# zengyan-97/X2-VLM

Measured on AMD Instinct MI355X. Metric: image-text pairs/sec (fwd+bwd) X2VLM-base 224px bs=64/GPU, higher is better.
Workload: dtype bf16

## Files before the change

### x2-vlm_amd/csrc/gemm.hip

```cpp
#include "x2_common.h"
#include <type_traits>

#define BM 128
#define BN 128
#define BK 64
#define TILE_BYTES (128 * 128)
#define STAGE_BYTES (2 * TILE_BYTES)
#define GEMM_LDS_BYTES (2 * STAGE_BYTES)

struct GemmNT {
  const bf16_t* A; const bf16_t* B; void* C;
  const float* bias; const float* gamma; const float* resid; bf16_t* aux;
  int M, N, K;
  int lda, ldb, ldc, ldr, ldaux;
  int act;
  int out_f32;
  int group_m;
  DropSpec drop;
  const uint32_t* drop_epoch;
  const float* rowscale;
  float* colsum;
  int dbg;
  int ksplit;
  const long* ce_labels;
// ... 1054 lines not shown
    const bool use64 = g_tune[3] == 3 || (g_tune[3] == 0 && (t128 <= slots || (t128 <= slots + slots / 6 && K <= 1024)));
    const bool use192 = !use64 && (g_tune[3] == 2 || (g_tune[3] == 0 && t128 > slots && t192 <= slots));
    const int t160 = ((M + 159) / 160) * ((N + BN - 1) / BN);
    const bool use160 = g_tune[3] == 4 || (use192 && g_tune[3] == 0 && t160 <= slots);
#define X2_NT_LAUNCH(V, SW)                                                                          \
    do {                                                                                              \
      if (use64) launch_nt<2, V, SW>(p, t64, (hipStream_t)stream);                                    \
      else if (use160) launch_nt<5, V, SW>(p, t160, (hipStream_t)stream);                             \
      else if (use192) launch_nt<6, V, SW>(p, t192, (hipStream_t)stream);                             \
      else launch_nt<4, V, SW>(p, t128, (hipStream_t)stream);                                         \
    } while (0)
    switch (var) {
      case 0: X2_NT_LAUNCH(0, false); break;
      case 2: X2_NT_LAUNCH(2, false); break;
      case 3: X2_NT_LAUNCH(3, false); break;
      case 1: X2_NT_LAUNCH(1, true); break;
      case 5: X2_NT_LAUNCH(5, true); break;
      case 6: X2_NT_LAUNCH(6, true); break;
      default: X2_NT_LAUNCH(4, false); break;
    }
#undef X2_NT_LAUNCH
  }
  return x2_check_launch("x2_gemm_nt");
}

extern "C" int x2_gemm_nt_dgelu_colparts(const void* A, const void* B, void* C, int M, int N, int K, int lda, int ldb, int ldc,
                                         const void* aux, int ldaux, float* colparts, int* nrows_out, void* stream) {
  X2_REQUIRE(A && B && C && aux && colparts && nrows_out, "x2_gemm_nt_dgelu_colparts: null argument");
  X2_REQUIRE(M > 0 && N > 0 && K > 0 && K % BK == 0 && N % 8 == 0, "x2_gemm_nt_dgelu_colparts: M=%d N=%d K=%d", M, N, K);
  X2_REQUIRE(lda % 8 == 0 && ldb % 8 == 0 && ldc % 8 == 0 && ldaux % 8 == 0, "x2_gemm_nt_dgelu_colparts: leading dims must keep 16-byte rows");
  GemmNT p{(const bf16_t*)A, (const bf16_t*)B, C, nullptr, nullptr, nullptr, (bf16_t*)aux, M, N, K, lda, ldb, ldc, 0, ldaux, 2, 0,
           g_tune[0] > 0 ? g_tune[0] : 8, DropSpec{0u, 0u, 1.f}, nullptr, nullptr, colparts, 0, 0};
  const int tiles_n = (N + BN - 1) / BN, t128 = ((M + 127) / 128) * tiles_n, t192 = ((M + 191) / 192) * tiles_n, t64 = ((M + 63) / 64) * tiles_n;
  const int slots = 2 * x2_cus();
  const bool use64 = g_tune[3] == 3 || (g_tune[3] == 0 && (t128 <= slots || (t128 <= slots + slots / 6 && K <= 1024)));
  const bool use192 = !use64 && (g_tune[3] == 2 || (g_tune[3] == 0 && t128 > slots && t192 <= slots));
  if (use64) { launch_nt<2, 10, false>(p, t64, (hipStream_t)stream); *nrows_out = 2 * ((M + 63) / 64); }
  else if (use192) { launch_nt<6, 10, false>(p, t192, (hipStream_t)stream); *nrows_out = 2 * ((M + 191) / 192); }
  else { launch_nt<4, 10, false>(p, t128, (hipStream_t)stream); *nrows_out = 2 * ((M + 127) / 128); }
  return x2_check_launch("x2_gemm_nt_dgelu_colparts");
}

__global__ __launch_bounds__(256) void gemm_nt_sum_slices_kernel(const float* __restrict__ ws, float* __restrict__ C, int M, int N, int ldc, int S) {
  const long e = (long)blockIdx.x * 256 + threadIdx.x, per = (long)M * N / 4;
  if (e >= per) return;
  const int m = (int)(e * 4 / N), n = (int)(e * 4 % N);
  float4 o = *reinterpret_cast<const float4*>(ws + e * 4);
  for (int s_ = 1; s_ < S; ++s_) {
    const float4 v = *reinterpret_cast<const float4*>(ws + (size_t)s_ * M * N + e * 4);
    o.x += v.x; o.y += v.y; o.z += v.z; o.w += v.w;
  }
  *reinterpret_cast<float4*>(C + (size_t)m * ldc + n) = o;
}
extern "C" int x2_gemm_nt_splitk(const void* A, const void* B, float* C, int M, int N, int K, int lda, int ldb, int ldc,
                                 int slices, float* ws, long ws_floats, void* stream) {
  X2_REQUIRE(A && B && C && M > 0 && N > 0 && K > 0, "x2_gemm_nt_splitk: empty problem M=%d N=%d K=%d", M, N, K);
  X2_REQUIRE(K % BK == 0 && N % 8 == 0, "x2_gemm_nt_splitk: K=%d must be a multiple of %d, N=%d of 8", K, BK, N);
  X2_REQUIRE(lda % 8 == 0 && ldb % 8 == 0 && ldc % 4 == 0 && ldc >= N, "x2_gemm_nt_splitk: leading dims must keep 16-byte rows");
  X2_REQUIRE(slices >= 0, "x2_gemm_nt_splitk: slices=%d", slices);
  const int nk = K / BK, tiles_n = (N + BN - 1) / BN;
  const bool small = M <= 64;
  const int tiles = (small ? (M + 63) / 64 : (M + 127) / 128) * tiles_n;
  int S = slices;
  if (S == 0) { S = (2 * x2_cus() + tiles - 1) / tiles; if (S > nk / 8) S = nk / 8; }
  if (S > nk) S = nk;
  const long per = (long)M * N;
  if (ws == nullptr) S = 1;
  else if ((long)S * per > ws_floats) S = (int)(ws_floats / per);
  if (S < 1) S = 1;
  const int steps = (nk + S - 1) / S;
  S = (nk + steps - 1) / steps;
  GemmNT p{(const bf16_t*)A, (const bf16_t*)B, S > 1 ? (void*)ws : (void*)C, nullptr, nullptr, nullptr, nullptr, M, N, K, lda, ldb,
           S > 1 ? N : ldc, 0, 0, 0, 1, g_tune[0] > 0 ? g_tune[0] : 8, DropSpec{0u, 0u, 1.f}, nullptr, nullptr, nullptr, 0, steps * BK};
  if (small) hipLaunchKernelGGL((gemm_nt_kernel<2, 7>), dim3(tiles, S), dim3(256), 2 * (64 * 128 + TILE_BYTES), (hipStream_t)stream, p);
  else hipLaunchKernelGGL((gemm_nt_kernel<4, 7>), dim3(tiles, S), dim3(256), GEMM_LDS_BYTES, (hipStream_t)stream, p);
  if (S > 1)
    hipLaunchKernelGGL(gemm_nt_sum_slices_kernel, dim3((unsigned)((per / 4 + 255) / 256)), dim3(256), 0, (hipStream_t)stream, ws, C, M, N, ldc, S);
  return x2_check_launch("x2_gemm_nt_splitk");
}

static int launch_nt_ce(GemmNT& p, int var, hipStream_t stream) {
  const int tiles_n = (p.N + BN - 1) / BN, t128 = ((p.M + 127) / 128) * tiles_n, t64 = ((p.M + 63) / 64) * tiles_n;
  const bool use64 = t128 <= 2 * x2_cus();
  if (var == 8) {
    if (use64) hipLaunchKernelGGL((gemm_nt_kernel<2, 8>), dim3(t64), dim3(256), 2 * (64 * 128 + TILE_BYTES), stream, p);
    else hipLaunchKernelGGL((gemm_nt_kernel<4, 8>), dim3(t128), dim3(256), GEMM_LDS_BYTES, stream, p);
  } else if (var == 11) {
    if (use64) hipLaunchKernelGGL((gemm_nt_kernel<2, 11>), dim3(t64), dim3(256), 2 * (64 * 128 + TILE_BYTES), stream, p);
    else hipLaunchKernelGGL((gemm_nt_kernel<4, 11>), dim3(t128), dim3(256), GEMM_LDS_BYTES, stream, p);
  } else if (var == 12) {
    if (use64) hipLaunchKernelGGL((gemm_nt_kernel<2, 12>), dim3(t64), dim3(256), 2 * (64 * 128 + TILE_BYTES), stream, p);
    else hipLaunchKernelGGL((gemm_nt_kernel<4, 12>), dim3(t128), dim3(256), GEMM_LDS_BYTES, stream, p);
  } else {
    if (use64) hipLaunchKernelGGL((gemm_nt_kernel<2, 9>), dim3(t64), dim3(256), 2 * (64 * 128 + TILE_BYTES), stream, p);
    else hipLaunchKernelGGL((gemm_nt_kernel<4, 9>), dim3(t128), dim3(256), GEMM_LDS_BYTES, stream, p);
  }
  return 0;
}
static bool mlm_ce_shapes_ok(int R, int Vp, int V, int Hd, int ldx, int lde) {
  return R > 0 && V > 0 && V <= Vp && Vp % 64 == 0 && Hd > 0 && Hd % BK == 0 && ldx % 8 == 0 && lde % 8 == 0 && ldx >= Hd && lde >= Hd;
}
extern "C" int x2_mlm_ce_fwd(const void* X, const void* E, const float* bias, const long* labels, int R, int Vp, int V, int Hd,
                             int ldx, int lde, float* part, float* zlab, void* stream) {
  X2_REQUIRE(X && E && labels && part && zlab, "x2_mlm_ce_fwd: null argument");
  X2_REQUIRE(mlm_ce_shapes_ok(R, Vp, V, Hd, ldx, lde), "x2_mlm_ce_fwd: R=%d Vp=%d V=%d Hd=%d ldx=%d lde=%d", R, Vp, V, Hd, ldx, lde);
  GemmNT p{(const bf16_t*)X, (const bf16_t*)E, nullptr, bias, nullptr, nullptr, nullptr, R, Vp, Hd, ldx, lde, Vp, 0, 0, 0, 0,
           g_tune[0] > 0 ? g_tune[0] : 8, DropSpec{0u, 0u, 1.f}, nullptr, nullptr, nullptr, 0, 0,
           labels, nullptr, nullptr, nullptr, part, zlab, 1.f, V};
  launch_nt_ce(p, 8, (hipStream_t)stream);
  return x2_check_launch("x2_mlm_ce_fwd");
}
extern "C" int x2_mlm_ce_bwd(const void* X, const void* E, const float* bias, const long* labels, const float* lse, const float* g,
                             const float* stat, float gscale, int R, int Vp, int V, int Hd, int ldx, int lde, void* dl_bf16, long ldd,
                             void* stream) {
  X2_REQUIRE(X && E && labels && lse && g && stat && dl_bf16, "x2_mlm_ce_bwd: null argument");
  X2_REQUIRE(mlm_ce_shapes_ok(R, Vp, V, Hd, ldx, lde) && ldd >= Vp && ldd % 8 == 0, "x2_mlm_ce_bwd: R=%d Vp=%d V=%d Hd=%d ldd=%ld", R, Vp, V, Hd, ldd);
  GemmNT p{(const bf16_t*)X, (const bf16_t*)E, dl_bf16, bias, nullptr, nullptr, nullptr, R, Vp, Hd, ldx, lde, (int)ldd, 0, 0, 0, 0,
           g_tune[0] > 0 ? g_tune[0] : 8, DropSpec{0u, 0u, 1.f}, nullptr, nullptr, nullptr, 0, 0,
           labels, lse, g, stat, nullptr, nullptr, gscale, V};
  launch_nt_ce(p, 9, (hipStream_t)stream);
  return x2_check_launch("x2_mlm_ce_bwd");
}
extern "C" int x2_mlm_ls_fwd(const void* X, const void* E, const float* bias, const long* labels, long ignore, int R, int Vp, int V, int Hd,
                             int ldx, int lde, float* part, float* sumz, float* zlab, float* zign, void* stream) {
  X2_REQUIRE(X && E && labels && part && sumz && zlab && zign, "x2_mlm_ls_fwd: null argument");
  X2_REQUIRE(mlm_ce_shapes_ok(R, Vp, V, Hd, ldx, lde) && V > 2 && ignore >= 0 && ignore < V,
             "x2_mlm_ls_fwd: R=%d Vp=%d V=%d Hd=%d ldx=%d lde=%d ignore=%ld", R, Vp, V, Hd, ldx, lde, ignore);
  GemmNT p{(const bf16_t*)X, (const bf16_t*)E, nullptr, bias, nullptr, nullptr, nullptr, R, Vp, Hd, ldx, lde, Vp, 0, 0, 0, 0,
           g_tune[0] > 0 ? g_tune[0] : 8, DropSpec{0u, 0u, 1.f}, nullptr, nullptr, nullptr, 0, 0,
           labels, nullptr, nullptr, nullptr, part, zlab, 1.f, V, sumz, zign, ignore, 0.f, nullptr};
  launch_nt_ce(p, 11, (hipStream_t)stream);
  return x2_check_launch("x2_mlm_ls_fwd");
}
extern "C" int x2_mlm_ls_bwd(const void* X, const void* E, const float* bias, const long* labels, const float* w, const float* lse, const float* g,
                             const float* stat, float gscale, float ls, long ignore, int R, int Vp, int V, int Hd, int ldx, int lde, void* dl_bf16,
                             long ldd, void* stream) {
  X2_REQUIRE(X && E && labels && w && lse && g && stat && dl_bf16, "x2_mlm_ls_bwd: null argument");
  X2_REQUIRE(mlm_ce_shapes_ok(R, Vp, V, Hd, ldx, lde) && ldd >= Vp && ldd % 8 == 0 && V > 2 && ignore >= 0 && ignore < V && ls >= 0.f && ls <= 1.f,
             "x2_mlm_ls_bwd: R=%d Vp=%d V=%d Hd=%d ldd=%ld ignore=%ld", R, Vp, V, Hd, ldd, ignore);
  GemmNT p{(const bf16_t*)X, (const bf16_t*)E, dl_bf16, bias, nullptr, nullptr, nullptr, R, Vp, Hd, ldx, lde, (int)ldd, 0, 0, 0, 0,
           g_tune[0] > 0 ? g_tune[0] : 8, DropSpec{0u, 0u, 1.f}, nullptr, nullptr, nullptr, 0, 0,
           labels, lse, g, stat, nullptr, nullptr, gscale, V, nullptr, nullptr, ignore, ls, w};
  launch_nt_ce(p, 12, (hipStream_t)stream);
  return x2_check_launch("x2_mlm_ls_bwd");
}

struct TNProblem {
  const bf16_t* A; const bf16_t* B; float* C;
  int Mc, N, K;
  int lda, ldb, ldc;
  int n_ld, k_ld;
  int tile_begin, tiles_k;
};
struct GemmTNGroup { TNProblem p[8]; int count; int accumulate; };

__device__ __forceinline__ int tn_f(int r) { return (r & 3) | (((r >> 3) & 1) << 2); }

__global__ __launch_bounds__(256, 2) void gemm_tn_kernel(GemmTNGroup g) {
  extern __shared__ __attribute__((aligned(16))) char smem[];
  const int tid = threadIdx.x, lane = tid & 63;
  const int wave = __builtin_amdgcn_readfirstlane(tid >> 6);
  const int wn = wave >> 1, wk = wave & 1;
  int t = xcd_remap(blockIdx.x, gridDim.x);
  int pi = 0;
#pragma unroll
  for (int i = 1; i < 8; ++i) if (i < g.count && t >= g.p[i].tile_begin) pi = i;
  const TNProblem p = g.p[pi];
  t -= p.tile_begin;
  int tnn, tkk;
  tile_coords(t, (p.N + 127) / 128, p.tiles_k, 8, tnn, tkk);
  const int n0 = tnn * 128, k0 = tkk * 128;
  const int steps = (p.Mc + BK - 1) / BK;
  const int per = (steps + gridDim.y - 1) / gridDim.y;
  const int s_begin = blockIdx.y * per, s_end = min(steps, s_begin + per);
  if (s_begin >= s_end) return;

  const bf16_t* srcA[4]; const bf16_t* srcB[4]; int rowq[4];
#pragma unroll
  for (int i = 0; i < 4; ++i) {
    const int q = i * 256 + tid, row = q >> 4, c = (q & 15) ^ (tn_f(row) << 1);
    int ca = n0 + c * 8; ca = ca <= p.n_ld - 8 ? ca : p.n_ld - 8;
    int cb = k0 + c * 8; cb = cb <= p.k_ld - 8 ? cb : p.k_ld - 8;
    rowq[i] = row;
    srcA[i] = p.A + (size_t)row * p.lda + ca;
    srcB[i] = p.B + (size_t)row * p.ldb + cb;
  }
  auto stage = [&](int s, int buf) {
    char* base = smem + buf * STAGE_BYTES;
    const int mbase = s * BK;
    if (mbase + BK <= p.Mc) {
#pragma unroll
      for (int i = 0; i < 4; ++i) {
        glds16(srcA[i] + (size_t)mbase * p.lda, base + (i * 256 + wave * 64) * 16);
        glds16(srcB[i] + (size_t)mbase * p.ldb, base + TILE_BYTES + (i * 256 + wave * 64) * 16);
      }
    } else {
#pragma unroll
      for (int i = 0; i < 4; ++i) {
        u32x4 va = u32x4{0, 0, 0, 0}, vb = u32x4{0, 0, 0, 0};
        if (mbase + rowq[i] < p.Mc) {
          va = *reinterpret_cast<const u32x4*>(srcA[i] + (size_t)mbase * p.lda);
          vb = *reinterpret_cast<const u32x4*>(srcB[i] + (size_t)mbase * p.ldb);
        }
        *reinterpret_cast<u32x4*>(base + (i * 256 + tid) * 16) = va;
        *reinterpret_cast<u32x4*>(base + TILE_BYTES + (i * 256 + tid) * 16) = vb;
      }
    }
  };

  f32x4 acc[4][4];
#pragma unroll
  for (int i = 0; i < 4; ++i)
#pragma unroll
    for (int j = 0; j < 4; ++j) acc[i][j] = f32x4{0.f, 0.f, 0.f, 0.f};

  const uint32_t lds0 = lds_addr(smem);
  const int fi = lane & 15, fg = lane >> 4, fr = fi >> 2, fc4 = fi & 3;
  const int fsw = (fr | ((fg & 1) << 2)) << 1;
  const uint32_t rowoff = (uint32_t)((fg * 8 + fr) * 256 + (fc4 & 1) * 8);

  stage(s_begin, 0);
  for (int s = s_begin; s < s_end; ++s) {
    const int it = s - s_begin;
    asm volatile("s_waitcnt vmcnt(0)" ::: "memory");
    __syncthreads();
    if (s + 1 < s_end) stage(s + 1, (it + 1) & 1);
    const uint32_t sb = lds0 + (it & 1) * STAGE_BYTES;
#pragma unroll
    for (int ks = 0; ks < 2; ++ks) {
      bf16x8 xa[4], ya[4];
#pragma unroll
      for (int i = 0; i < 4; ++i) {
        const uint32_t ch = (uint32_t)(((2 * (wk * 4 + i) + (fc4 >> 1)) ^ fsw) << 4);
        const uint32_t a0 = sb + TILE_BYTES + ks * 32 * 256 + rowoff + ch;
        xa[i] = lds_read_tr_frag(a0, a0 + 4 * 256);
      }
#pragma unroll
      for (int j = 0; j < 4; ++j) {
        const uint32_t ch = (uint32_t)(((2 * (wn * 4 + j) + (fc4 >> 1)) ^ fsw) << 4);
        const uint32_t a0 = sb + ks * 32 * 256 + rowoff + ch;
        ya[j] = lds_read_tr_frag(a0, a0 + 4 * 256);
      }
#pragma unroll
      for (int i = 0; i < 4; ++i)
#pragma unroll
        for (int j = 0; j < 4; ++j)
          acc[i][j] = __builtin_amdgcn_mfma_f32_16x16x32_bf16(xa[i], ya[j], acc[i][j], 0, 0, 0);
    }
  }

  const bool atomic = gridDim.y > 1;
#pragma unroll
  for (int j = 0; j < 4; ++j) {
    const int n = n0 + wn * 64 + j * 16 + fi;
    if (n >= p.N) continue;
#pragma unroll
    for (int i = 0; i < 4; ++i) {
      const int k = k0 + wk * 64 + i * 16 + fg * 4;
      if (k >= p.K) continue;
      float* dst = p.C + (size_t)n * p.ldc + k;
      if (atomic) {
#pragma unroll
        for (int r = 0; r < 4; ++r) atomicAdd(dst + r, acc[i][j][r]);
      } else if (g.accumulate) {
        float4 o = *reinterpret_cast<float4*>(dst);
        o.x += acc[i][j][0]; o.y += acc[i][j][1]; o.z += acc[i][j][2]; o.w += acc[i][j][3];
        *reinterpret_cast<float4*>(dst) = o;
      } else {
        *reinterpret_cast<float4*>(dst) = float4{acc[i][j][0], acc[i][j][1], acc[i][j][2], acc[i][j][3]};
      }
    }
  }
}

#define T2_HALF 16384
#define T2_LDS_BYTES (8 * T2_HALF)
__device__ __attribute__((aligned(16))) const uint32_t x2_zero_chunk[4] = {0u, 0u, 0u, 0u};
template <bool RAG>
__global__ __launch_bounds__(512) void gemm_tn256_kernel(GemmTNGroup g, float* ws, int total_tiles) {
  extern __shared__ __attribute__((aligned(16))) char smem[];
  const int tid = threadIdx.x, lane = tid & 63;
  const int wave = __builtin_amdgcn_readfirstlane(tid >> 6);
  const int wr = wave >> 2, wc = wave & 3;
  const int tile = xcd_remap(blockIdx.x, gridDim.x);
  int pi = 0;
#pragma unroll
  for (int i = 1; i < 8; ++i) if (i < g.count && tile >= g.p[i].tile_begin) pi = i;
  const TNProblem p = g.p[pi];
  int tnn, tkk;
  tile_coords(tile - p.tile_begin, (p.N + 255) / 256, p.tiles_k, 4, tnn, tkk);
  const int n0 = tnn * 256, k0 = tkk * 256;
  const int steps = (p.Mc + BK - 1) / BK, rag = p.Mc % BK;
  const int s_begin = (int)((long)steps * blockIdx.y / gridDim.y), s_end = (int)((long)steps * (blockIdx.y + 1) / gridDim.y);
  const int nk = s_end - s_begin;
  const int last_rel = (RAG && rag != 0 && s_end == steps) ? nk - 1 : -1;
  const bf16_t* const zsrc = reinterpret_cast<const bf16_t*>(x2_zero_chunk);
  const bool oob0 = (tid >> 4) >= rag, oob1 = ((512 + tid) >> 4) >= rag;

  const bf16_t* srcA[2][2]; const bf16_t* srcB[2][2];
#pragma unroll
  for (int h = 0; h < 2; ++h)
#pragma unroll
    for (int i = 0; i < 2; ++i) {
      const int q = i * 512 + tid, row = q >> 4, c = (q & 15) ^ (tn_f(row) << 1);
      int ca = n0 + h * 128 + c * 8; ca = ca <= p.n_ld - 8 ? ca : p.n_ld - 8;
      int cb = k0 + h * 128 + c * 8; cb = cb <= p.k_ld - 8 ? cb : p.k_ld - 8;
      srcA[h][i] = p.A + ((size_t)s_begin * BK + row) * p.lda + ca;
      srcB[h][i] = p.B + ((size_t)s_begin * BK + row) * p.ldb + cb;
    }
  const size_t stepA = (size_t)BK * p.lda, stepB = (size_t)BK * p.ldb;
  auto issue = [&](int kt, auto slot) {
    constexpr int S = decltype(slot)::value;
    char* base = smem + ((kt & 1) * 4 + S) * T2_HALF + wave * 1024;
    const bool z = RAG && kt == last_rel;
    if constexpr (S < 2) {
      glds16(z && oob0 ? zsrc : srcA[S][0] + kt * stepA, base);
      glds16(z && oob1 ? zsrc : srcA[S][1] + kt * stepA, base + 8192);
    } else {
      glds16(z && oob0 ? zsrc : srcB[S - 2][0] + kt * stepB, base);
      glds16(z && oob1 ? zsrc : srcB[S - 2][1] + kt * stepB, base + 8192);
    }
  };
  using S0 = std::integral_constant<int, 0>; using S1 = std::integral_constant<int, 1>;
  using S2 = std::integral_constant<int, 2>; using S3 = std::integral_constant<int, 3>;

  f32x4 acc[4][8];
#pragma unroll
  for (int i = 0; i < 4; ++i)
#pragma unroll
    for (int j = 0; j < 8; ++j) acc[i][j] = f32x4{0.f, 0.f, 0.f, 0.f};

  const uint32_t lds0 = lds_addr(smem);
  const int fi = lane & 15, fg = lane >> 4, fr = fi >> 2, fc4 = fi & 3;
  const int fsw = (fr | ((fg & 1) << 2)) << 1;
  const uint32_t rowoff = (uint32_t)((fg * 8 + fr) * 256 + (fc4 & 1) * 8);
  const uint32_t offA = (uint32_t)(wr * T2_HALF) + rowoff, offB = (uint32_t)((2 + (wc >> 1)) * T2_HALF) + rowoff;
  bf16x8 fa[2][4], fb[2][4];
  auto readA = [&](uint32_t buf, int jh) {
#pragma unroll
    for (int ks = 0; ks < 2; ++ks)
#pragma unroll
      for (int j = 0; j < 4; ++j) {
        const uint32_t a0 = buf + offA + ks * 8192 + (uint32_t)(((2 * (jh * 4 + j) + (fc4 >> 1)) ^ fsw) << 4);
        fa[ks][j] = lds_read_tr_frag_async(a0, a0 + 1024);
      }
  };
  auto readB = [&](uint32_t buf, int ih) {
#pragma unroll
    for (int ks = 0; ks < 2; ++ks)
#pragma unroll
      for (int i = 0; i < 2; ++i) {
        const uint32_t a0 = buf + offB + ks * 8192 + (uint32_t)(((2 * ((wc & 1) * 4 + ih * 2 + i) + (fc4 >> 1)) ^ fsw) << 4);
        fb[ks][ih * 2 + i] = lds_read_tr_frag_async(a0, a0 + 1024);
      }
  };
  auto quad = [&](auto jh_, auto ih_) {
    constexpr int jh = decltype(jh_)::value, ih = decltype(ih_)::value;
#pragma unroll
    for (int ks = 0; ks < 2; ++ks)
#pragma unroll
      for (int j = 0; j < 4; ++j)
#pragma unroll
        for (int i = 0; i < 2; ++i)
          acc[ih * 2 + i][jh * 4 + j] = __builtin_amdgcn_mfma_f32_16x16x32_bf16(fb[ks][ih * 2 + i], fa[ks][j], acc[ih * 2 + i][jh * 4 + j], 0, 0, 0);
  };
#define T2_FENCE() __builtin_amdgcn_sched_barrier(0)
  auto ktile = [&](int kt, auto n1_, auto n2_) {
    constexpr bool n1 = decltype(n1_)::value, n2 = decltype(n2_)::value;
    const uint32_t buf = lds0 + (uint32_t)((kt & 1) * 4 * T2_HALF);
    readA(buf, 0); readB(buf, 0); readB(buf, 1);
    if constexpr (n1) issue(kt + 1, S0{});
    asm volatile("s_waitcnt lgkmcnt(8)" ::: "memory"); T2_FENCE();
    quad(S0{}, S0{}); T2_FENCE();
    if constexpr (n1) issue(kt + 1, S1{});
    asm volatile("s_waitcnt lgkmcnt(0)" ::: "memory"); T2_FENCE();
    quad(S0{}, S1{}); T2_FENCE();
    if constexpr (n2) { asm volatile("s_barrier" ::: "memory"); issue(kt + 2, S2{}); }
    readA(buf, 1);
    asm volatile("s_waitcnt lgkmcnt(0)" ::: "memory"); T2_FENCE();
    quad(S1{}, S1{}); T2_FENCE();
    if constexpr (n2) issue(kt + 2, S3{});
    quad(S1{}, S0{}); T2_FENCE();
    if constexpr (n1) {
      if constexpr (n2) asm volatile("s_waitcnt vmcnt(4)\n\ts_barrier" ::: "memory");
      else asm volatile("s_waitcnt vmcnt(0)\n\ts_barrier" ::: "memory");
      T2_FENCE();
    }
  };
  issue(0, S0{}); issue(0, S1{}); issue(0, S2{}); issue(0, S3{});
  if (nk > 1) { issue(1, S2{}); issue(1, S3{}); asm volatile("s_waitcnt vmcnt(4)\n\ts_barrier" ::: "memory"); }
  else asm volatile("s_waitcnt vmcnt(0)\n\ts_barrier" ::: "memory");
  int kt = 0;
  for (; kt + 2 < nk; ++kt) ktile(kt, std::true_type{}, std::true_type{});
  if (kt + 1 < nk) { ktile(kt, std::true_type{}, std::false_type{}); ++kt; }
  ktile(kt, std::false_type{}, std::false_type{});

  if (gridDim.y > 1) {
    float* dst = ws + ((size_t)blockIdx.y * total_tiles + tile) * 65536 + (size_t)wave * 8192 + lane * 4;
#pragma unroll
    for (int i = 0; i < 4; ++i)
#pragma unroll
      for (int j = 0; j < 8; ++j)
        *reinterpret_cast<float4*>(dst + (i * 8 + j) * 256) = float4{acc[i][j][0], acc[i][j][1], acc[i][j][2], acc[i][j][3]};
    return;
  }
#pragma unroll
  for (int j = 0; j < 8; ++j) {
    const int n = n0 + wr * 128 + j * 16 + fi;
    if (n >= p.N) continue;
#pragma unroll
    for (int i = 0; i < 4; ++i) {
      const int k = k0 + wc * 64 + i * 16 + fg * 4;
      if (k >= p.K) continue;
      float* dst = p.C + (size_t)n * p.ldc + k;
      float4 o = float4{acc[i][j][0], acc[i][j][1], acc[i][j][2], acc[i][j][3]};
      if (g.accumulate) { const float4 c = *reinterpret_cast<float4*>(dst); o.x += c.x; o.y += c.y; o.z += c.z; o.w += c.w; }
      *reinterpret_cast<float4*>(dst) = o;
    }
  }
}
__global__ __launch_bounds__(256) void gemm_tn256_reduce_kernel(GemmTNGroup g, const float* __restrict__ ws, int total_tiles, int split) {
  const int tile = blockIdx.x >> 6;
  int pi = 0;
#pragma unroll
  for (int i = 1; i < 8; ++i) if (i < g.count && tile >= g.p[i].tile_begin) pi = i;
  const TNProblem p = g.p[pi];
  int tnn, tkk;
  tile_coords(tile - p.tile_begin, (p.N + 255) / 256, p.tiles_k, 4, tnn, tkk);
  const int e = (blockIdx.x & 63) * 256 + threadIdx.x;
  const int lane = e & 63, ij = (e >> 6) & 31, wave = e >> 11;
  const int i = ij >> 3, j = ij & 7, fi = lane & 15, fg = lane >> 4, wr = wave >> 2, wc = wave & 3;
  const int n = tnn * 256 + wr * 128 + j * 16 + fi, k = tkk * 256 + wc * 64 + i * 16 + fg * 4;
  const float* src = ws + (size_t)tile * 65536 + (size_t)e * 4;
  float4 o = *reinterpret_cast<const float4*>(src);
  for (int s_ = 1; s_ < split; ++s_) {
    const float4 v = *reinterpret_cast<const float4*>(src + (size_t)s_ * total_tiles * 65536);
    o.x += v.x; o.y += v.y; o.z += v.z; o.w += v.w;
  }
  if (n >= p.N || k >= p.K) return;
  float* dst = p.C + (size_t)n * p.ldc + k;
  if (g.accumulate) { const float4 c = *reinterpret_cast<float4*>(dst); o.x += c.x; o.y += c.y; o.z += c.z; o.w += c.w; }
  *reinterpret_cast<float4*>(dst) = o;
}

extern "C" int x2_gemm_tn_grouped(const int64_t* problems, int count, int accumulate, int split, float* ws, long ws_floats,
                                  void* stream) {
  X2_REQUIRE(count >= 1 && count <= 8, "x2_gemm_tn_grouped: count=%d not in [1,8]", count);
  X2_REQUIRE(split >= 0, "x2_gemm_tn_grouped: split=%d", split);
  GemmTNGroup g; g.count = count; g.accumulate = accumulate;
  int tiles = 0, tiles256 = 0, min_steps = 1 << 30;
  bool big = g_tune[5] != 1;
  for (int i = 0; i < count; ++i) {
    const int64_t* q = problems + i * 11;
    TNProblem& p = g.p[i];
    p.A = (const bf16_t*)q[0]; p.B = (const bf16_t*)q[1]; p.C = (float*)q[2];
    p.Mc = (int)q[3]; p.N = (int)q[4]; p.K = (int)q[5]; p.lda = (int)q[6]; p.ldb = (int)q[7]; p.ldc = (int)q[8];
    p.n_ld = (int)q[9]; p.k_ld = (int)q[10];
    X2_REQUIRE(p.Mc > 0 && p.N > 0 && p.K > 0, "x2_gemm_tn_grouped[%d]: empty problem", i);
    X2_REQUIRE(p.K % 4 == 0 && p.ldc % 4 == 0, "x2_gemm_tn_grouped[%d]: K, ldc must be multiples of 4", i);
    X2_REQUIRE(p.lda % 8 == 0 && p.ldb % 8 == 0 && p.n_ld % 8 == 0 && p.k_ld % 8 == 0 && p.n_ld >= 8 && p.k_ld >= 8,
               "x2_gemm_tn_grouped[%d]: rows must be 16-byte granular", i);
    X2_REQUIRE(p.n_ld <= p.lda && p.k_ld <= p.ldb, "x2_gemm_tn_grouped[%d]: n_ld/k_ld exceed leading dims", i);
    tiles += ((p.N + 127) / 128) * ((p.K + 127) / 128);
    tiles256 += ((p.N + 255) / 256) * ((p.K + 255) / 256);
    const int steps_i = (p.Mc + BK - 1) / BK;
    min_steps = steps_i < min_steps ? steps_i : min_steps;
  }
  if (g_tune[5] != 2 && tiles256 < 24 && !(split > 1 && ws)) big = false;
  if (big) {
    int t = 0;
    for (int i = 0; i < count; ++i) { g.p[i].tile_begin = t; g.p[i].tiles_k = (g.p[i].K + 255) / 256; t += ((g.p[i].N + 255) / 256) * g.p[i].tiles_k; }
    const int cus = x2_cus();
    int sp = split;
    if (sp == 0) {
      double best = -1.0; sp = 1;
      for (int c = 1; c <= 4 && min_steps / c >= 16; ++c) {
        const long blocks = (long)t * c;
        const double fill = (double)blocks / (double)(((blocks + cus - 1) / cus) * cus);
        if (fill > best + 0.03) { best = fill; sp = c; }
      }
    }
    while (sp > 1 && (sp > min_steps || !ws || (long)sp * t * 65536 > ws_floats)) --sp;
    static bool attr = false;
    if (!attr) {
      (void)hipFuncSetAttribute(reinterpret_cast<const void*>(gemm_tn256_kernel<false>), hipFuncAttributeMaxDynamicSharedMemorySize, T2_LDS_BYTES);
      (void)hipFuncSetAttribute(reinterpret_cast<const void*>(gemm_tn256_kernel<true>), hipFuncAttributeMaxDynamicSharedMemorySize, T2_LDS_BYTES);
      attr = true;
    }
    bool ragged = false;
    for (int i = 0; i < count; ++i) ragged = ragged || (g.p[i].Mc % BK != 0);
    if (ragged) hipLaunchKernelGGL(gemm_tn256_kernel<true>, dim3(t, sp), dim3(512), T2_LDS_BYTES, (hipStream_t)stream, g, ws, t);
    else hipLaunchKernelGGL(gemm_tn256_kernel<false>, dim3(t, sp), dim3(512), T2_LDS_BYTES, (hipStream_t)stream, g, ws, t);
    if (sp > 1) hipLaunchKernelGGL(gemm_tn256_reduce_kernel, dim3(t * 64), dim3(256), 0, (hipStream_t)stream, g, ws, t, sp);
    return x2_check_launch("x2_gemm_tn_grouped");
  }
  if (split == 0) split = 1;
  X2_REQUIRE(split == 1 || accumulate, "x2_gemm_tn_grouped: split>1 on the 128x128 kernel adds atomically: pass accumulate=1 and a defined C");
  int t = 0;
  for (int i = 0; i < count; ++i) { g.p[i].tile_begin = t; g.p[i].tiles_k = (g.p[i].K + 127) / 128; t += ((g.p[i].N + 127) / 128) * g.p[i].tiles_k; }
  hipLaunchKernelGGL(gemm_tn_kernel, dim3(t, split), dim3(256), GEMM_LDS_BYTES, (hipStream_t)stream, g);
  return x2_check_launch("x2_gemm_tn_grouped");
}
```

### x2-vlm_amd/csrc/x2_common.h

```cpp
#pragma once
#include <hip/hip_runtime.h>
#include <stdint.h>

typedef uint16_t bf16_t;
typedef __attribute__((ext_vector_type(8))) short bf16x8;
typedef __attribute__((ext_vector_type(4))) short bf16x4;
typedef __attribute__((ext_vector_type(4))) float f32x4;
typedef __attribute__((ext_vector_type(4))) uint32_t u32x4;
typedef __attribute__((ext_vector_type(2))) uint32_t u32x2;

#define X2_OK 0
#define X2_ERR_ARG (-1)
#define X2_ERR_LAUNCH (-2)

void x2_set_error(const char* fmt, ...);
int x2_check_launch(const char* what);

#define X2_REQUIRE(cond, ...) do { if (!(cond)) { x2_set_error(__VA_ARGS__); return X2_ERR_ARG; } } while (0)

__device__ __forceinline__ float bf2f(bf16_t h) { return __uint_as_float(((uint32_t)h) << 16); }
__device__ __forceinline__ bf16_t f2bf(float f) {
  uint32_t u = __float_as_uint(f);
  u += 0x7fffu + ((u >> 16) & 1u);
  return (bf16_t)(u >> 16);
}
__device__ __forceinline__ uint32_t pack_bf16(float a, float b) {
  uint32_t r;
  asm volatile("v_cvt_pk_bf16_f32 %0, %1, %2" : "=v"(r) : "v"(a), "v"(b));
  return r;
}
__device__ __forceinline__ float bf_lo(uint32_t u) { return __uint_as_float(u << 16); }
__device__ __forceinline__ float bf_hi(uint32_t u) { return __uint_as_float(u & 0xffff0000u); }

__device__ __forceinline__ float gelu_tail(float ax, float e) {
  const float t = __builtin_amdgcn_rcpf(fmaf(ax, 0.3275911f * 0.70710678118654752f, 1.0f));
  const float poly = t * (0.127414796f + t * (-0.142248368f + t * (0.7107068705f + t * (-0.7265760135f + t * 0.5307027145f))));
  return poly * e;
}
__device__ __forceinline__ float gelu_f(float x) {
  const float ax = fabsf(x);
  const float h = gelu_tail(ax, __builtin_amdgcn_exp2f(x * x * -0.72134752044448170f));
  return fmaf(-ax, h, fmaxf(x, 0.0f));
}
__device__ __forceinline__ float dgelu_f(float x) {
  const float e = __builtin_amdgcn_exp2f(x * x * -0.72134752044448170f);
  const float h = gelu_tail(fabsf(x), e);
  return fmaf(x * 0.3989422804014327f, e, x >= 0.0f ? 1.0f - h : h);
}

struct DropSpec { uint32_t thr16; uint32_t seed; float scale; };
__device__ __forceinline__ uint32_t x2_hash(uint32_t x) {
  x ^= x >> 16; x *= 0x7feb352dU; x ^= x >> 15; x *= 0x846ca68bU; x ^= x >> 16;
  return x;
}
__device__ __forceinline__ DropSpec drop_at_epoch(DropSpec d, const uint32_t* __restrict__ epoch) {
  if (epoch) d.seed = x2_hash(d.seed + 0x9E3779B1u * epoch[0]);
  return d;
}
__device__ __forceinline__ float drop_mul(const DropSpec& d, uint32_t e) {
  const uint32_t h = x2_hash((e >> 1) ^ d.seed);
  const uint32_t u = (e & 1u) ? (h >> 16) : (h & 0xffffu);
  return u >= d.thr16 ? d.scale : 0.f;
}
__device__ __forceinline__ void drop_mul4(const DropSpec& d, uint32_t e0, float m[4]) {
  const uint32_t h0 = x2_hash((e0 >> 1) ^ d.seed), h1 = x2_hash(((e0 >> 1) + 1u) ^ d.seed);
  m[0] = (h0 & 0xffffu) >= d.thr16 ? d.scale : 0.f;
  m[1] = (h0 >> 16) >= d.thr16 ? d.scale : 0.f;
  m[2] = (h1 & 0xffffu) >= d.thr16 ? d.scale : 0.f;
  m[3] = (h1 >> 16) >= d.thr16 ? d.scale : 0.f;
}
__device__ __forceinline__ float wave_sum(float v) {
#pragma unroll
  for (int o = 32; o > 0; o >>= 1) v += __shfl_xor(v, o, 64);
  return v;
}
__device__ __forceinline__ float wave_max(float v) {
#pragma unroll
  for (int o = 32; o > 0; o >>= 1) v = fmaxf(v, __shfl_xor(v, o, 64));
  return v;
}

__device__ __forceinline__ uint32_t lds_addr(const void* p) { return (uint32_t)(uintptr_t)p; }

__device__ __forceinline__ bf16x8 lds_read_b128(uint32_t byte_addr) {
  return *reinterpret_cast<const __attribute__((address_space(3))) bf16x8*>((uintptr_t)byte_addr);
}
__device__ __forceinline__ bf16x4 lds_read_tr64(uint32_t byte_addr) {
  return __builtin_amdgcn_ds_read_tr16_b64_v4i16(
      (__attribute__((address_space(3))) bf16x4*)(uintptr_t)byte_addr);
}
__device__ __forceinline__ bf16x8 lds_read_tr_frag(uint32_t a0, uint32_t a1) {
  const bf16x4 lo = lds_read_tr64(a0), hi = lds_read_tr64(a1);
  return __builtin_shufflevector(lo, hi, 0, 1, 2, 3, 4, 5, 6, 7);
}
__device__ __forceinline__ bf16x8 lds_read_tr_frag_async(uint32_t a0, uint32_t a1) {
  bf16x4 lo, hi;
  asm volatile("ds_read_b64_tr_b16 %0, %1" : "=v"(lo) : "v"(a0));
  asm volatile("ds_read_b64_tr_b16 %0, %1" : "=v"(hi) : "v"(a1));
  return __builtin_shufflevector(lo, hi, 0, 1, 2, 3, 4, 5, 6, 7);
}
__device__ __forceinline__ void lds_wait_all() { asm volatile("s_waitcnt lgkmcnt(0)" ::: "memory"); }

__device__ __forceinline__ void glds16(const void* gptr, void* lds_base) {
  __builtin_amdgcn_global_load_lds((const __attribute__((address_space(1))) void*)gptr,
                                   (__attribute__((address_space(3))) void*)lds_base, 16, 0, 0);
}

__device__ __forceinline__ int xcd_remap(int bid, int nwg) {
  const int q = nwg >> 3, r = nwg & 7, xcd = bid & 7, idx = bid >> 3;
  return (xcd < r ? xcd * (q + 1) : r * (q + 1) + (xcd - r) * q) + idx;
}
```

Before: 2953.

## Restructure TN256 weight-gradient main loop with finer-grained LDS read/MFMA interleaving

Rewrites the 256x256 TN gemm main loop into a two-step parity-unrolled schedule. Fragment reads are interleaved per MFMA group with graduated lgkmcnt waits, and the next tile's fragments are prefetched across the step boundary. LDS layout changes from per-stage to per-slot with parity offsets folded into immediate ds_read offsets. Global source pointers become 32-bit byte offsets off a single base, which requires leading dims up to 2^24. Probe-only ablation hooks and timing scripts are added. The goal is less LDS-read latency exposure and lower address arithmetic, at the cost of more intricate wait counts and code size.

```diff
diff --git a/probes/cmp_tn_builds.py b/probes/cmp_tn_builds.py
--- /dev/null
+++ b/probes/cmp_tn_builds.py
@@ -0,0 +1,109 @@
+import argparse
+import importlib
+import json
+import os
+import sys
+
+sys.path.insert(0, os.path.dirname(os.path.dirname(os.path.abspath(__file__))))
+import numpy as np
+
+NSETS, PASSES, ROUNDS = 3, 4, 3
+
+
+def layer(rows, D):
+    return [(rows, D, 4 * D), (rows, 4 * D, D), (rows, D, D), (rows, 3 * D, D)]
+
+
+LAUNCHES = {
+    "vision_pair": (layer(12608, 768) * 2, 0),
+    "text_pair": (layer(3840, 768) * 2, 0),
+    "fusion_pair": ((layer(7680, 768) + [(7680, 768, 768), (12608, 1536, 768), (7680, 768, 768)]) * 2, 0),
+    "large_pair": (layer(18464, 1024) * 2, 0),
+    "patch_embed": ([(12544, 768, 768)], 8),
+}
+
+
+def same(a, b):
+    names = sorted(os.listdir(a))
+    assert names == sorted(os.listdir(b)) and names, "different file lists"
+    bad = 0
+    for n in names:
+        x, y = np.load(os.path.join(a, n)), np.load(os.path.join(b, n))
+        eq = x.shape == y.shape and np.array_equal(x.view(np.uint8), y.view(np.uint8))
+        bad += 0 if eq else 1
+        print("%-44s %s" % (n, "identical" if eq else "DIFFERENT"))
+    print("%d files, %d differ" % (len(names), bad))
+    return bad == 0
+
+
+def table(a_files, b_files):
+    def best(files):
+        runs = [json.load(open(f)) for f in files]
+        return {k: min(r[k]["us"] for r in runs) for k in runs[0]}, runs[0]
+    (a, meta), (b, _) = best(a_files), best(b_files)
+    print("%-14s %9s %9s %9s %8s   %8s %8s" % ("launch", "GFLOP", "A us", "B us", "B / A", "A TF/s", "B TF/s"))
+    for k in a:
+        gf = meta[k]["gflop"]
+        print("%-14s %9.1f %9.1f %9.1f %8.3f   %8.0f %8.0f" % (k, gf, a[k], b[k], b[k] / a[k], gf / a[k] * 1e3, gf / b[k] * 1e3))
+
+
+def main():
+    ap = argparse.ArgumentParser()
+    ap.add_argument("--dump")
+    ap.add_argument("--json")
+    ap.add_argument("--same", nargs=2)
+    ap.add_argument("--table", nargs=2)
+    args = ap.parse_args()
+    if args.same:
+        sys.exit(0 if same(*args.same) else 1)
+    if args.table:
+        return table(args.table[0].split(","), args.table[1].split(","))
+
+    import torch
+    K = importlib.import_module("x2-vlm_amd.kernels")
+    dev = "cuda"
+    gen = torch.Generator(device=dev).manual_seed(1234)
+
+    def rnd(*shape):
+        return torch.randn(*shape, generator=gen, device=dev).to(torch.bfloat16)
+
+    sets = {k: [[(rnd(Mc, N), rnd(Mc, Kd), torch.empty(N, Kd, device=dev)) for Mc, N, Kd in probs] for _ in range(NSETS)] for k, (probs, _) in LAUNCHES.items()}
+    launches = {k: (lambda i, k=k: K.gemm_tn_grouped(sets[k][i % NSETS], split=LAUNCHES[k][1])) for k in LAUNCHES}
+    gflop = {k: sum(2.0 * Mc * N * Kd for Mc, N, Kd in probs) / 1e9 for k, (probs, _) in LAUNCHES.items()}
+
+    if args.dump:
+        os.makedirs(args.dump, exist_ok=True)
+        for k, (probs, split) in LAUNCHES.items():
+            chunks = [probs[i:i + 8] for i in range(0, len(probs), 8)]
+            want = max((split if split else 4) * sum(((N + 255) // 256) * ((Kd + 255) // 256) for _, N, Kd in c) * 65536 for c in chunks)
+            ws = K.workspace(torch.device(dev, torch.cuda.current_device()), want)
+            ws[:want].zero_()
+            launches[k](0)
+            torch.cuda.synchronize()
+            for j, p in enumerate(sets[k][0]):
+                np.save(os.path.join(args.dump, "%s.%02d.dW.npy" % (k, j)), p[2].cpu().numpy())
+            if bool(ws[:want].any()):
+                np.save(os.path.join(args.dump, "%s.ws.npy" % k), ws[:want].cpu().numpy())
+
+    best = {k: float("inf") for k in launches}
+    for k, f in launches.items():
+        f(0)
+    torch.cuda.synchronize()
+    for _ in range(ROUNDS):
+        for k, f in launches.items():
+            a, e = torch.cuda.Event(enable_timing=True), torch.cuda.Event(enable_timing=True)
+            a.record()
+            for i in range(NSETS * PASSES):
+                f(i)
+            e.record()
+            torch.cuda.synchronize()
+            best[k] = min(best[k], a.elapsed_time(e) * 1e3 / (NSETS * PASSES))
+    res = {k: {"us": best[k], "gflop": gflop[k]} for k in launches}
+    for k, v in res.items():
+        print("%-14s %8.1f us  %8.1f GFLOP  %6.0f TFLOP/s" % (k, v["us"], v["gflop"], v["gflop"] / v["us"] * 1e3))
+    if args.json:
+        json.dump(res, open(args.json, "w"))
+
+
+if __name__ == "__main__":
+    main()
diff --git a/probes/tn_loop_ablation.py b/probes/tn_loop_ablation.py
--- /dev/null
+++ b/probes/tn_loop_ablation.py
@@ -0,0 +1,41 @@
+import ctypes, importlib, os, sys
+sys.path.insert(0, os.path.dirname(os.path.dirname(os.path.abspath(__file__))))
+import torch
+K = importlib.import_module("x2-vlm_amd.kernels")
+lib = importlib.import_module("x2-vlm_amd._lib").lib()
+tuned = importlib.import_module("x2-vlm_amd._lib").tuned
+assert hasattr(lib, "x2_probe_set_buffer"), "needs the probe build"
+lib.x2_probe_set_buffer.argtypes, lib.x2_probe_set_buffer.restype = [ctypes.c_void_p], ctypes.c_int
+dev = "cuda"
+NSET = 4
+LAYER = [(768, 3072), (3072, 768), (768, 768), (2304, 768)]
+VARIANTS = [("all three", 0), ("no DMA", 32), ("no reads", 64), ("no MFMA", 128), ("MFMA only", 32 + 64), ("reads only", 32 + 128), ("DMA only", 64 + 128)]
+for name, Mc in (("vision pair", 12608), ("text pair", 3840)):
+    sets = [[(torch.randn(Mc, N, device=dev).bfloat16(), torch.randn(Mc, Kd, device=dev).bfloat16(), torch.empty(N, Kd, device=dev))
+             for N, Kd in LAYER * 2] for _ in range(NSET)]
+    steps = (Mc + 63) // 64
+    nbuf = torch.zeros(4096 * 4, device=dev, dtype=torch.int64)
+    res = []
+    for vname, bits in VARIANTS:
+        with tuned({5: 2, 2: bits}):
+            for s in sets:
+                K.gemm_tn_grouped(s, split=1)
+            torch.cuda.synchronize()
+            mains, spans = [], []
+            for rep in range(2 * NSET):
+                nbuf.zero_()
+                lib.x2_probe_set_buffer(ctypes.c_void_p(nbuf.data_ptr()))
+                a, e = torch.cuda.Event(enable_timing=True), torch.cuda.Event(enable_timing=True)
+                a.record()
+                K.gemm_tn_grouped(sets[rep % NSET], split=1)
+                e.record()
+                torch.cuda.synchronize()
+                lib.x2_probe_set_buffer(None)
+                t = nbuf.view(-1, 4).cpu().double()
+                t = t[t[:, 2] > 0] / 100.0
+                mains.append(float((t[:, 2] - t[:, 1]).mean()))
+                spans.append(a.elapsed_time(e) * 1e3)
+        res.append((vname, min(mains), min(spans)))
+    print("%-11s 8 problems, Mc=%d (%d contraction steps per 256 x 256 tile, 216 tiles)" % (name, Mc, steps))
+    for vname, m, sp in res:
+        print("   %-12s main loop %7.2f us per tile = %5.2f us per step   launch %6.1f us" % (vname, m, m / steps, sp))
diff --git a/x2-vlm_amd/csrc/gemm.hip b/x2-vlm_amd/csrc/gemm.hip
--- a/x2-vlm_amd/csrc/gemm.hip
+++ b/x2-vlm_amd/csrc/gemm.hip
@@ -1230,7 +1230,21 @@
   int n_ld, k_ld;
   int tile_begin, tiles_k;
 };
+#ifdef X2_PROBE
+struct GemmTNGroup { TNProblem p[8]; int count; int accumulate; int dbg; };
+#define TN_ABL_DECL(g) const bool abl_dma_ = ((g).dbg & 32) != 0, abl_rd_ = ((g).dbg & 64) != 0, abl_mm_ = ((g).dbg & 128) != 0
+#define TN_ABL_NO_DMA(kt) if (abl_dma_ && (kt) >= 2) return
+#define TN_ABL_NO_READ(kt) if (abl_rd_ && (kt) >= 1) return
+#define TN_ABL_NO_MFMA() if (abl_mm_) return
+#define TN_STAMP(i) do { if (g_nt_probe && threadIdx.x == 0) g_nt_probe[((size_t)blockIdx.y * gridDim.x + blockIdx.x) * 4 + (i)] = wall_clock64(); } while (0)
+#else
 struct GemmTNGroup { TNProblem p[8]; int count; int accumulate; };
+#define TN_ABL_DECL(g)
+#define TN_ABL_NO_DMA(kt)
+#define TN_ABL_NO_READ(kt)
+#define TN_ABL_NO_MFMA()
+#define TN_STAMP(i) do { } while (0)
+#endif
 
 __device__ __forceinline__ int tn_f(int r) { return (r & 3) | (((r >> 3) & 1) << 2); }
 
@@ -1372,10 +1386,10 @@
   const int s_begin = (int)((long)steps * blockIdx.y / gridDim.y), s_end = (int)((long)steps * (blockIdx.y + 1) / gridDim.y);
   const int nk = s_end - s_begin;
   const int last_rel = (RAG && rag != 0 && s_end == steps) ? nk - 1 : -1;
-  const bf16_t* const zsrc = reinterpret_cast<const bf16_t*>(x2_zero_chunk);
+  const char* const zsrc0 = reinterpret_cast<const char*>(x2_zero_chunk);
   const bool oob0 = (tid >> 4) >= rag, oob1 = ((512 + tid) >> 4) >= rag;
 
-  const bf16_t* srcA[2][2]; const bf16_t* srcB[2][2];
+  uint32_t offA[2][2], offB[2][2];
 #pragma unroll
   for (int h = 0; h < 2; ++h)
 #pragma unroll
@@ -1383,24 +1397,32 @@
       const int q = i * 512 + tid, row = q >> 4, c = (q & 15) ^ (tn_f(row) << 1);
       int ca = n0 + h * 128 + c * 8; ca = ca <= p.n_ld - 8 ? ca : p.n_ld - 8;
       int cb = k0 + h * 128 + c * 8; cb = cb <= p.k_ld - 8 ? cb : p.k_ld - 8;
-      srcA[h][i] = p.A + ((size_t)s_begin * BK + row) * p.lda + ca;
-      srcB[h][i] = p.B + ((size_t)s_begin * BK + row) * p.ldb + cb;
-    }
-  const size_t stepA = (size_t)BK * p.lda, stepB = (size_t)BK * p.ldb;
-  auto issue = [&](int kt, auto slot) {
-    constexpr int S = decltype(slot)::value;
-    char* base = smem + ((kt & 1) * 4 + S) * T2_HALF + wave * 1024;
-    const bool z = RAG && kt == last_rel;
-    if constexpr (S < 2) {
-      glds16(z && oob0 ? zsrc : srcA[S][0] + kt * stepA, base);
-      glds16(z && oob1 ? zsrc : srcA[S][1] + kt * stepA, base + 8192);
+      offA[h][i] = (uint32_t)(row * p.lda + ca) * 2u;
+      offB[h][i] = (uint32_t)(row * p.ldb + cb) * 2u;
+    }
+  const char* const baseA = reinterpret_cast<const char*>(p.A + (size_t)s_begin * BK * p.lda);
+  const char* const baseB = reinterpret_cast<const char*>(p.B + (size_t)s_begin * BK * p.ldb);
+  const size_t stepA = (size_t)BK * p.lda * 2, stepB = (size_t)BK * p.ldb * 2;
+  TN_ABL_DECL(g);
+  TN_STAMP(0);
+  using C0 = std::integral_constant<int, 0>; using C1 = std::integral_constant<int, 1>;
+  using C2 = std::integral_constant<int, 2>; using C3 = std::integral_constant<int, 3>;
+  auto issue = [&](int kt, auto par_, auto slot, auto rz_) {
+    constexpr int S = decltype(slot)::value, par = decltype(par_)::value;
+    constexpr bool rz = decltype(rz_)::value;
+    TN_ABL_NO_DMA(kt);
+    char* base = smem + (S * 2 + par) * T2_HALF + wave * 1024;
+    const char* const src = S < 2 ? baseA + kt * stepA : baseB + kt * stepB;
+    uint32_t o0 = S < 2 ? offA[S & 1][0] : offB[S & 1][0], o1 = S < 2 ? offA[S & 1][1] : offB[S & 1][1];
+    asm("" : "+v"(o0), "+v"(o1));
+    if (RAG && rz && kt == last_rel) {
+      glds16(oob0 ? zsrc0 : src + o0, base);
+      glds16(oob1 ? zsrc0 : src + o1, base + 8192);
     } else {
-      glds16(z && oob0 ? zsrc : srcB[S - 2][0] + kt * stepB, base);
-      glds16(z && oob1 ? zsrc : srcB[S - 2][1] + kt * stepB, base + 8192);
-    }
-  };
-  using S0 = std::integral_constant<int, 0>; using S1 = std::integral_constant<int, 1>;
-  using S2 = std::integral_constant<int, 2>; using S3 = std::integral_constant<int, 3>;
+      glds16(src + o0, base);
+      glds16(src + o1, base + 8192);
+    }
+  };
 
   f32x4 acc[4][8];
 #pragma unroll
@@ -1412,66 +1434,93 @@
   const int fi = lane & 15, fg = lane >> 4, fr = fi >> 2, fc4 = fi & 3;
   const int fsw = (fr | ((fg & 1) << 2)) << 1;
   const uint32_t rowoff = (uint32_t)((fg * 8 + fr) * 256 + (fc4 & 1) * 8);
-  const uint32_t offA = (uint32_t)(wr * T2_HALF) + rowoff, offB = (uint32_t)((2 + (wc >> 1)) * T2_HALF) + rowoff;
+  uint32_t aA[8], aB[4];
+#pragma unroll
+  for (int j = 0; j < 8; ++j) aA[j] = lds0 + (uint32_t)(wr * 2 * T2_HALF) + rowoff + (uint32_t)(((2 * j + (fc4 >> 1)) ^ fsw) << 4);
+#pragma unroll
+  for (int i = 0; i < 4; ++i)
+    aB[i] = lds0 + (uint32_t)((2 + (wc >> 1)) * 2 * T2_HALF) + rowoff + (uint32_t)(((2 * ((wc & 1) * 4 + i) + (fc4 >> 1)) ^ fsw) << 4);
   bf16x8 fa[2][4], fb[2][4];
-  auto readA = [&](uint32_t buf, int jh) {
+  auto readA = [&](int kt, auto par_, auto jh_, auto j_) {
+    constexpr int par = decltype(par_)::value, jh = decltype(jh_)::value, j = decltype(j_)::value;
+    TN_ABL_NO_READ(kt);
+    fa[0][j] = lds_read_tr_frag_async_off<par * T2_HALF>(aA[jh * 4 + j]);
+    fa[1][j] = lds_read_tr_frag_async_off<par * T2_HALF + 8192>(aA[jh * 4 + j]);
+  };
+  auto readB = [&](int kt, auto par_, auto ih_, auto i_) {
+    constexpr int par = decltype(par_)::value, t = decltype(ih_)::value * 2 + decltype(i_)::value;
+    TN_ABL_NO_READ(kt);
+    fb[0][t] = lds_read_tr_frag_async_off<par * T2_HALF>(aB[t]);
+    fb[1][t] = lds_read_tr_frag_async_off<par * T2_HALF + 8192>(aB[t]);
+  };
+  auto mm = [&](auto jh_, auto ih_, auto j_) {
+    constexpr int jh = decltype(jh_)::value, ih = decltype(ih_)::value, j = decltype(j_)::value;
+    TN_ABL_NO_MFMA();
 #pragma unroll
     for (int ks = 0; ks < 2; ++ks)
 #pragma unroll
-      for (int j = 0; j < 4; ++j) {
-        const uint32_t a0 = buf + offA + ks * 8192 + (uint32_t)(((2 * (jh * 4 + j) + (fc4 >> 1)) ^ fsw) << 4);
-        fa[ks][j] = lds_read_tr_frag_async(a0, a0 + 1024);
-      }
-  };
-  auto readB = [&](uint32_t buf, int ih) {
-#pragma unroll
-    for (int ks = 0; ks < 2; ++ks)
-#pragma unroll
-      for (int i = 0; i < 2; ++i) {
-        const uint32_t a0 = buf + offB + ks * 8192 + (uint32_t)(((2 * ((wc & 1) * 4 + ih * 2 + i) + (fc4 >> 1)) ^ fsw) << 4);
-        fb[ks][ih * 2 + i] = lds_read_tr_frag_async(a0, a0 + 1024);
-      }
-  };
-  auto quad = [&](auto jh_, auto ih_) {
-    constexpr int jh = decltype(jh_)::value, ih = decltype(ih_)::value;
-#pragma unroll
-    for (int ks = 0; ks < 2; ++ks)
-#pragma unroll
-      for (int j = 0; j < 4; ++j)
-#pragma unroll
-        for (int i = 0; i < 2; ++i)
-          acc[ih * 2 + i][jh * 4 + j] = __builtin_amdgcn_mfma_f32_16x16x32_bf16(fb[ks][ih * 2 + i], fa[ks][j], acc[ih * 2 + i][jh * 4 + j], 0, 0, 0);
+      for (int i = 0; i < 2; ++i)
+        acc[ih * 2 + i][jh * 4 + j] = __builtin_amdgcn_mfma_f32_16x16x32_bf16(fb[ks][ih * 2 + i], fa[ks][j], acc[ih * 2 + i][jh * 4 + j], 0, 0, 0);
   };
 #define T2_FENCE() __builtin_amdgcn_sched_barrier(0)
-  auto ktile = [&](int kt, auto n1_, auto n2_) {
-    constexpr bool n1 = decltype(n1_)::value, n2 = decltype(n2_)::value;
-    const uint32_t buf = lds0 + (uint32_t)((kt & 1) * 4 * T2_HALF);
-    readA(buf, 0); readB(buf, 0); readB(buf, 1);
-    if constexpr (n1) issue(kt + 1, S0{});
-    asm volatile("s_waitcnt lgkmcnt(8)" ::: "memory"); T2_FENCE();
-    quad(S0{}, S0{}); T2_FENCE();
-    if constexpr (n1) issue(kt + 1, S1{});
-    asm volatile("s_waitcnt lgkmcnt(0)" ::: "memory"); T2_FENCE();
-    quad(S0{}, S1{}); T2_FENCE();
-    if constexpr (n2) { asm volatile("s_barrier" ::: "memory"); issue(kt + 2, S2{}); }
-    readA(buf, 1);
-    asm volatile("s_waitcnt lgkmcnt(0)" ::: "memory"); T2_FENCE();
-    quad(S1{}, S1{}); T2_FENCE();
-    if constexpr (n2) issue(kt + 2, S3{});
-    quad(S1{}, S0{}); T2_FENCE();
-    if constexpr (n1) {
-      if constexpr (n2) asm volatile("s_waitcnt vmcnt(4)\n\ts_barrier" ::: "memory");
+#define T2_LGKM(n) do { asm volatile("s_waitcnt lgkmcnt(" #n ")" ::: "memory"); T2_FENCE(); } while (0)
+  auto head_reads_b = [&](int kt, auto par_, auto f_) { readB(kt, par_, f_, C0{}); readB(kt, par_, f_, C1{}); T2_FENCE(); };
+  auto step = [&](int kt, auto par_, auto n1_, auto n2_, auto rz_) {
+    constexpr int P = decltype(par_)::value;
+    const bool n1 = n1_, n2 = n2_;
+    using PP = std::integral_constant<int, P>; using PN = std::integral_constant<int, 1 - P>;
+    using F = std::integral_constant<int, P>; using S = std::integral_constant<int, 1 - P>;
+    if (n1) { issue(kt + 1, PN{}, C1{}, rz_); T2_FENCE(); }
+    T2_LGKM(12); mm(C0{}, F{}, C0{}); T2_FENCE();
+    readB(kt, PP{}, S{}, C0{}); T2_FENCE();
+    T2_LGKM(12); mm(C0{}, F{}, C1{}); T2_FENCE();
+    readB(kt, PP{}, S{}, C1{}); T2_FENCE();
+    T2_LGKM(12); mm(C0{}, F{}, C2{}); T2_FENCE();
+    T2_LGKM(8); mm(C0{}, F{}, C3{}); T2_FENCE();
+    T2_LGKM(0); mm(C0{}, S{}, C0{}); T2_FENCE();
+    readA(kt, PP{}, C1{}, C0{}); T2_FENCE();
+    mm(C0{}, S{}, C1{}); T2_FENCE();
+    readA(kt, PP{}, C1{}, C1{}); T2_FENCE();
+    mm(C0{}, S{}, C2{}); T2_FENCE();
+    readA(kt, PP{}, C1{}, C2{}); T2_FENCE();
+    mm(C0{}, S{}, C3{}); T2_FENCE();
+    readA(kt, PP{}, C1{}, C3{}); T2_FENCE();
+    if (n2) { asm volatile("s_barrier" ::: "memory"); T2_FENCE(); issue(kt + 2, PP{}, C2{}, rz_); T2_FENCE(); }
+    T2_LGKM(12); mm(C1{}, S{}, C0{}); T2_FENCE();
+    T2_LGKM(8); mm(C1{}, S{}, C1{}); T2_FENCE();
+    T2_LGKM(4); mm(C1{}, S{}, C2{}); T2_FENCE();
+    T2_LGKM(0); mm(C1{}, S{}, C3{}); T2_FENCE();
+    if (n1) {
+      if (n2) asm volatile("s_waitcnt vmcnt(2)\n\ts_barrier" ::: "memory");
       else asm volatile("s_waitcnt vmcnt(0)\n\ts_barrier" ::: "memory");
       T2_FENCE();
-    }
-  };
-  issue(0, S0{}); issue(0, S1{}); issue(0, S2{}); issue(0, S3{});
-  if (nk > 1) { issue(1, S2{}); issue(1, S3{}); asm volatile("s_waitcnt vmcnt(4)\n\ts_barrier" ::: "memory"); }
+      if (n2) { issue(kt + 2, PP{}, C0{}, rz_); issue(kt + 2, PP{}, C3{}, rz_); T2_FENCE(); }
+      head_reads_b(kt + 1, PN{}, S{});
+    }
+    mm(C1{}, F{}, C0{}); T2_FENCE();
+    if (n1) { readA(kt + 1, PN{}, C0{}, C0{}); T2_FENCE(); }
+    mm(C1{}, F{}, C1{}); T2_FENCE();
+    if (n1) { readA(kt + 1, PN{}, C0{}, C1{}); T2_FENCE(); }
+    mm(C1{}, F{}, C2{}); T2_FENCE();
+    if (n1) { readA(kt + 1, PN{}, C0{}, C2{}); T2_FENCE(); }
+    mm(C1{}, F{}, C3{}); T2_FENCE();
+    if (n1) { readA(kt + 1, PN{}, C0{}, C3{}); T2_FENCE(); }
+  };
+  using T = std::true_type; using N = std::false_type;
+  issue(0, C0{}, C0{}, T{}); issue(0, C0{}, C1{}, T{}); issue(0, C0{}, C2{}, T{}); issue(0, C0{}, C3{}, T{});
+  if (nk > 1) { issue(1, C1{}, C2{}, T{}); issue(1, C1{}, C3{}, T{}); issue(1, C1{}, C0{}, T{}); asm volatile("s_waitcnt vmcnt(6)\n\ts_barrier" ::: "memory"); }
   else asm volatile("s_waitcnt vmcnt(0)\n\ts_barrier" ::: "memory");
+  T2_FENCE();
+  TN_STAMP(1);
+  head_reads_b(0, C0{}, C0{});
+  readA(0, C0{}, C0{}, C0{}); readA(0, C0{}, C0{}, C1{}); readA(0, C0{}, C0{}, C2{}); readA(0, C0{}, C0{}, C3{}); T2_FENCE();
   int kt = 0;
-  for (; kt + 2 < nk; ++kt) ktile(kt, std::true_type{}, std::true_type{});
-  if (kt + 1 < nk) { ktile(kt, std::true_type{}, std::false_type{}); ++kt; }
-  ktile(kt, std::false_type{}, std::false_type{});
+  for (; kt + 3 + (RAG ? 1 : 0) < nk; kt += 2) { step(kt, C0{}, T{}, T{}, N{}); step(kt + 1, C1{}, T{}, T{}, N{}); }
+  for (; kt < nk; kt += 2) {
+    step(kt, C0{}, kt + 1 < nk, kt + 2 < nk, T{});
+    if (kt + 1 < nk) step(kt + 1, C1{}, kt + 2 < nk, kt + 3 < nk, T{});
+  }
+  TN_STAMP(2);
 
   if (gridDim.y > 1) {
     float* dst = ws + ((size_t)blockIdx.y * total_tiles + tile) * 65536 + (size_t)wave * 8192 + lane * 4;
@@ -1526,6 +1575,9 @@
   X2_REQUIRE(count >= 1 && count <= 8, "x2_gemm_tn_grouped: count=%d not in [1,8]", count);
   X2_REQUIRE(split >= 0, "x2_gemm_tn_grouped: split=%d", split);
   GemmTNGroup g; g.count = count; g.accumulate = accumulate;
+#ifdef X2_PROBE
+  g.dbg = g_tune[2];
+#endif
   int tiles = 0, tiles256 = 0, min_steps = 1 << 30;
   bool big = g_tune[5] != 1;
   for (int i = 0; i < count; ++i) {
@@ -1539,6 +1591,7 @@
     X2_REQUIRE(p.lda % 8 == 0 && p.ldb % 8 == 0 && p.n_ld % 8 == 0 && p.k_ld % 8 == 0 && p.n_ld >= 8 && p.k_ld >= 8,
                "x2_gemm_tn_grouped[%d]: rows must be 16-byte granular", i);
     X2_REQUIRE(p.n_ld <= p.lda && p.k_ld <= p.ldb, "x2_gemm_tn_grouped[%d]: n_ld/k_ld exceed leading dims", i);
+    X2_REQUIRE(p.lda <= (1 << 24) && p.ldb <= (1 << 24), "x2_gemm_tn_grouped[%d]: leading dimension above 2^24", i);
     tiles += ((p.N + 127) / 128) * ((p.K + 127) / 128);
     tiles256 += ((p.N + 255) / 256) * ((p.K + 255) / 256);
     const int steps_i = (p.Mc + BK - 1) / BK;
diff --git a/x2-vlm_amd/csrc/x2_common.h b/x2-vlm_amd/csrc/x2_common.h
--- a/x2-vlm_amd/csrc/x2_common.h
+++ b/x2-vlm_amd/csrc/x2_common.h
@@ -99,6 +99,14 @@
   asm volatile("ds_read_b64_tr_b16 %0, %1" : "=v"(hi) : "v"(a1));
   return __builtin_shufflevector(lo, hi, 0, 1, 2, 3, 4, 5, 6, 7);
 }
+template <int OFF>
+__device__ __forceinline__ bf16x8 lds_read_tr_frag_async_off(uint32_t a) {
+  static_assert(OFF >= 0 && OFF + 1024 < 65536, "ds_read offset field is 16 bits");
+  bf16x4 lo, hi;
+  asm volatile("ds_read_b64_tr_b16 %0, %1 offset:%2" : "=v"(lo) : "v"(a), "n"(OFF));
+  asm volatile("ds_read_b64_tr_b16 %0, %1 offset:%2" : "=v"(hi) : "v"(a), "n"(OFF + 1024));
+  return __builtin_shufflevector(lo, hi, 0, 1, 2, 3, 4, 5, 6, 7);
+}
 __device__ __forceinline__ void lds_wait_all() { asm volatile("s_waitcnt lgkmcnt(0)" ::: "memory"); }
 
 __device__ __forceinline__ void glds16(const void* gptr, void* lds_base) {
```

Result: no change. 2978 (median of 6 runs) (+0.9%).
